# MCG-NJU/MeMOTR

Hardware: AMD Instinct MI355X
Metric: train_frames_per_sec (higher is better)
Workload: dtype f32

## Files before the change

### include/clip_ops_hip.h

```cpp
#ifndef CLIP_OPS_HIP_H
#define CLIP_OPS_HIP_H

#include <stdint.h>

#ifdef __cplusplus
extern "C" {
#endif

#define CLIPOPS_ABI_VERSION 12

int clipops_abi_version(void);
const char *clipops_last_error(void);

int clipops_match_cost_f32(const float *logits, long logit_sl, long logit_sq, const float *boxes, long box_sl,
                           long box_sq, const int64_t *gt_labels, const float *gt_boxes, int n_layers, int Q, int K,
                           int T, float w_class, float w_bbox, float w_giou, float *cost, void *stream);

int clipops_pair_box_loss_fwd_f32(const float *boxes, const int64_t *lay, const int64_t *qidx, long row_mul,
                                  long row_add, const float *tgt_boxes, const int64_t *gidx, const float *weight,
                                  int n, float *l1, float *giou_loss, void *stream);
int clipops_pair_box_loss_bwd_f32(const float *boxes, const int64_t *lay, const int64_t *qidx, long row_mul,
                                  long row_add, const float *tgt_boxes, const int64_t *gidx, const float *weight,
                                  int n, const float *grad_l1, const float *grad_giou, float *grad_boxes,
                                  void *stream);
// ... 55 lines not shown

#define CLIPOPS_ASSIGN_MAX_DIM 2048
int clipops_assign_f32(const float *cost, long stride_problem, long stride_row, long stride_col, int n_problems,
                       int n_rows, int n_cols, int32_t *row_ind, int32_t *col_ind, int32_t *status, void *stream);

int clipops_shift_relu_f32(float *x, const float *shift, const float *res, long planes, int C, long HW, void *stream);
int clipops_shift_relu_bf16(uint16_t *x, const float *shift, const uint16_t *res, long planes, int C, long HW,
                            void *stream);

int clipops_linear_bwd_f32(const float *grad_y, const float *y_relu, const float *x, const float *w, int rows,
                           int in_features, int out_features, float *grad_x, float *grad_w, float *grad_b,
                           void *stream);

int clipops_linear_fwd_f32(const float *x, const float *w, const float *bias, int rows, int in_features,
                           int out_features, int relu, float *y, void *stream);

int clipops_relu_bwd_colsum_partial_f32(const float *g, const float *y, long rows, int cols, int chunk_rows, float *g2,
                                        float *partial, void *stream);

int clipops_result_rows_f32(const float *boxes, const float *scores, const int64_t *ids, const int64_t *labels, int n,
                            int K, int64_t frame, float ori_w, float ori_h, float score_thresh, float area_thresh,
                            float *rows_f, int64_t *rows_i, int32_t *counters, int capacity, void *stream);

#ifdef __cplusplus
}
#endif
#endif
```

### memotr_amd/_clip_lib.py

```python
from __future__ import annotations

import ctypes

from . import _cabi

LIB_PATH = _cabi.lib_path("libclip_ops_hip.so")

ABI_VERSION = 12

c_int, c_long, c_float, c_void_p = ctypes.c_int, ctypes.c_long, ctypes.c_float, ctypes.c_void_p

_PAIR = [c_void_p, c_void_p, c_void_p, c_long, c_long, c_void_p, c_void_p, c_void_p, c_int]
_FOCAL = [c_void_p, c_long, c_long, c_void_p, c_int, c_int, c_int, c_float, c_float]

SYMBOLS = {
    "clipops_abi_version": ([], c_int),
    "clipops_last_error": ([], ctypes.c_char_p),
    "clipops_match_cost_f32": ([c_void_p, c_long, c_long, c_void_p, c_long, c_long, c_void_p, c_void_p] + [c_int] * 4 +
                               [c_float] * 3 + [c_void_p, c_void_p], c_int),
    "clipops_pair_box_loss_fwd_f32": (_PAIR + [c_void_p, c_void_p, c_void_p], c_int),
    "clipops_pair_box_loss_bwd_f32": (_PAIR + [c_void_p, c_void_p, c_void_p, c_void_p], c_int),
    "clipops_pair_iou_f32": ([c_void_p, c_void_p, c_void_p, c_int, c_void_p, c_void_p], c_int),
    "clipops_track_ownership_i64": ([c_void_p, c_int, c_void_p, c_int, c_void_p, c_void_p, c_void_p], c_int),
    "clipops_focal_labels_i64": ([c_void_p, c_void_p, c_void_p, c_int, c_void_p, c_int, c_void_p, c_int, c_void_p, c_int,
# ... 9 lines not shown
                                                                                          c_void_p], c_int),
    "clipops_mha_bwd_f32": ([c_void_p] * 3 + [c_long] * 6 + [c_void_p] * 4 + [c_int] * 3 + [c_float] +
                            [c_void_p, c_long, c_long] * 3 + [c_void_p], c_int),
    "clipops_add_layer_norm_fwd_f32": ([c_void_p] * 4 + [c_long, c_float] + [c_void_p] * 4, c_int),
    "clipops_add_layer_norm_bwd_f32": ([c_void_p] * 4 + [c_long, c_int] + [c_void_p] * 3, c_int),
    "clipops_add_layer_norm_pos_fwd_f32": ([c_void_p] * 5 + [c_long, c_float] + [c_void_p] * 5, c_int),
    "clipops_add_layer_norm_fanin_bwd_f32": ([c_void_p] * 6 + [c_long, c_int] + [c_void_p] * 4, c_int),
    "clipops_sine_embed_fwd_f32": ([c_void_p, c_void_p, c_long, c_int, c_int, c_float, c_void_p, c_void_p], c_int),
    "clipops_sine_embed_bwd_f32": ([c_void_p, c_void_p, c_long, c_int, c_int, c_float, c_void_p, c_void_p, c_void_p],
                                   c_int),
    "clipops_inverse_sigmoid_fwd_f32": ([c_void_p, c_long, c_float, c_void_p, c_void_p], c_int),
    "clipops_inverse_sigmoid_bwd_f32": ([c_void_p, c_void_p, c_long, c_float, c_void_p, c_void_p], c_int),
    "clipops_refine_boxes_fwd_f32": ([c_void_p, c_void_p, c_long, c_float, c_void_p, c_void_p], c_int),
    "clipops_linear_bwd_f32": ([c_void_p] * 4 + [c_int] * 3 + [c_void_p] * 4, c_int),
    "clipops_linear_fwd_f32": ([c_void_p] * 3 + [c_int] * 4 + [c_void_p, c_void_p], c_int),
    "clipops_relu_bwd_colsum_partial_f32": ([c_void_p, c_void_p, c_long, c_int, c_int, c_void_p, c_void_p, c_void_p], c_int),
    "clipops_shift_relu_f32": ([c_void_p, c_void_p, c_void_p, c_long, c_int, c_long, c_void_p], c_int),
    "clipops_shift_relu_bf16": ([c_void_p, c_void_p, c_void_p, c_long, c_int, c_long, c_void_p], c_int),
    "clipops_refine_boxes_bwd_f32": ([c_void_p, c_void_p, c_void_p, c_long, c_float, c_void_p, c_void_p, c_void_p],
                                     c_int),
    "clipops_refine_boxes_split_fwd_f32": ([c_void_p, c_void_p, c_long, c_float, c_void_p, c_void_p, c_void_p], c_int),
    "clipops_result_rows_f32": ([c_void_p] * 4 + [c_int, c_int, ctypes.c_int64] + [c_float] * 4 + [c_void_p] * 3 +
                                [c_int, c_void_p], c_int),
}


lib, check = _cabi.bind("libclip_ops_hip.so", "clipops", SYMBOLS, ABI_VERSION)
```

### memotr_amd/csrc/clip_ops.hip

```cpp
#include <hip/hip_runtime.h>
#include <stdint.h>
#include <stdio.h>

#include <atomic>

#include "../../include/clip_ops_hip.h"
#include "assign_core.h"

namespace {

thread_local char g_err[256] = {0};

int fail(int code, const char *msg) {
    snprintf(g_err, sizeof(g_err), "%s", msg);
    return code;
}

int check_launch(const char *what) {
    const hipError_t e = hipGetLastError();
    if (e != hipSuccess) {
        snprintf(g_err, sizeof(g_err), "%s: %s", what, hipGetErrorString(e));
        return (int)e;
    }
    g_err[0] = 0;
// ... 69 lines not shown
                                                               const int64_t *__restrict__ lay,
                                                               const int64_t *__restrict__ qidx, long row_mul,
                                                               long row_add, const float *__restrict__ tgt,
                                                               const int64_t *__restrict__ gidx,
                                                               const float *__restrict__ weight, int n,
                                                               float *__restrict__ l1, float *__restrict__ gl) {
#pragma clang fp contract(off)
    const int i = blockIdx.x * blockDim.x + threadIdx.x;
    if (i >= n) return;
    const float *pb = boxes + (lay[i] * row_mul + row_add + qidx[i]) * 4;
    const float *tb = tgt + (gidx ? gidx[i] : (long)i) * 4;
    const float p0 = pb[0], p1 = pb[1], p2 = pb[2], p3 = pb[3];
    const float t0 = tb[0], t1 = tb[1], t2 = tb[2], t3 = tb[3];
    float a = ((fabsf(p0 - t0) + fabsf(p1 - t1)) + fabsf(p2 - t2)) + fabsf(p3 - t3);
    float g = 1.f - giou_pair(to_xyxy(p0, p1, p2, p3), to_xyxy(t0, t1, t2, t3));
    if (weight) {
        a *= weight[i];
        g *= weight[i];
    }
    l1[i] = a;
    gl[i] = g;
}

__global__ __launch_bounds__(256) void pair_iou_kernel(const float *__restrict__ boxes, const float *__restrict__ tgt,
                                                      const int64_t *__restrict__ gidx, int n,
                                                      float *__restrict__ iou) {
#pragma clang fp contract(off)
    const int i = blockIdx.x * blockDim.x + threadIdx.x;
    if (i >= n) return;
    const float *pb = boxes + (long)i * 4;
    const float *tb = tgt + (gidx ? gidx[i] : (long)i) * 4;
    const Box a = to_xyxy(pb[0], pb[1], pb[2], pb[3]), b = to_xyxy(tb[0], tb[1], tb[2], tb[3]);
    const float iw = fmaxf(fminf(a.x2, b.x2) - fmaxf(a.x1, b.x1), 0.f);
    const float ih = fmaxf(fminf(a.y2, b.y2) - fmaxf(a.y1, b.y1), 0.f);
    const float inter = iw * ih;
    const float uni = (a.x2 - a.x1) * (a.y2 - a.y1) + (b.x2 - b.x1) * (b.y2 - b.y1) - inter;
    iou[i] = inter / uni;
}

__device__ __forceinline__ float dmax_a(float a, float b) { return a > b ? 1.f : (a == b ? 0.5f : 0.f); }
__device__ __forceinline__ float dmin_a(float a, float b) { return a < b ? 1.f : (a == b ? 0.5f : 0.f); }
__device__ __forceinline__ float sgn(float x) { return x > 0.f ? 1.f : (x < 0.f ? -1.f : 0.f); }

__global__ __launch_bounds__(256) void pair_box_loss_bwd_kernel(const float *__restrict__ boxes,
                                                               const int64_t *__restrict__ lay,
                                                               const int64_t *__restrict__ qidx, long row_mul,
                                                               long row_add, const float *__restrict__ tgt,
                                                               const int64_t *__restrict__ gidx,
                                                               const float *__restrict__ weight, int n,
                                                               const float *__restrict__ g_l1,
                                                               const float *__restrict__ g_gl,
                                                               float *__restrict__ grad_boxes) {
    const int i = blockIdx.x * blockDim.x + threadIdx.x;
    if (i >= n) return;
    const long row = lay[i] * row_mul + row_add + qidx[i];
    const float *pb = boxes + row * 4;
    const float *tb = tgt + (gidx ? gidx[i] : (long)i) * 4;
    const float p0 = pb[0], p1 = pb[1], p2 = pb[2], p3 = pb[3];
    const float t0 = tb[0], t1 = tb[1], t2 = tb[2], t3 = tb[3];
    const float w = weight ? weight[i] : 1.f;
// ... 1091 lines not shown
int clipops_focal_labels_i64(const int64_t *lay, const int64_t *q, const int64_t *g, int n_pairs,
                             const int64_t *gt_labels, int n_gt, const int64_t *matched_idx, int n_tracks,
                             const uint8_t *late, int n_layers, int n_det, int K, int64_t *labels, void *stream) {
    if (n_pairs < 0 || n_gt < 0 || n_tracks < 0 || n_layers < 0 || n_det < 0) return fail(1, "clipops_focal_labels_i64: negative count");
    if ((long)n_layers * (n_det + n_tracks) == 0) { g_err[0] = 0; return 0; }
    if (!labels || !late || (n_pairs > 0 && (!lay || !q || !g || !gt_labels)) || (n_tracks > 0 && !matched_idx) ||
        (n_gt > 0 && !gt_labels))
        return fail(1, "clipops_focal_labels_i64: null pointer");
    hipLaunchKernelGGL(focal_labels_kernel, dim3(1), dim3(256), 0, (hipStream_t)stream, lay, q, g, n_pairs, gt_labels, n_gt,
                       matched_idx, n_tracks, late, n_layers, n_det, K, labels);
    return check_launch("focal_labels_kernel");
}

int clipops_pair_iou_f32(const float *boxes, const float *tgt_boxes, const int64_t *gidx, int n, float *iou,
                         void *stream) {
    if (n < 0) return fail(1, "clipops_pair_iou_f32: negative count");
    if (n == 0) { g_err[0] = 0; return 0; }
    if (!boxes || !tgt_boxes || !iou) return fail(1, "clipops_pair_iou_f32: null pointer");
    hipLaunchKernelGGL(pair_iou_kernel, dim3((n + 255) / 256), dim3(256), 0, (hipStream_t)stream, boxes, tgt_boxes,
                       gidx, n, iou);
    return check_launch("pair_iou_kernel");
}

int clipops_focal_fwd_f32(const float *logits, long sl, long sq, const int64_t *labels, int n_layers, int Nq, int K,
                          float alpha, float gamma, float *loss, void *stream) {
    if (n_layers < 0 || Nq < 0 || K <= 0) return fail(1, "clipops_focal_fwd_f32: bad dimension");
    if (n_layers == 0) { g_err[0] = 0; return 0; }
    if (!loss || (Nq > 0 && (!logits || !labels))) return fail(1, "clipops_focal_fwd_f32: null pointer");
    hipLaunchKernelGGL(focal_fwd_kernel, dim3(n_layers), dim3(256), 0, (hipStream_t)stream, logits, sl, sq, labels, Nq,
                       K, alpha, gamma, loss);
    return check_launch("focal_fwd_kernel");
}

int clipops_focal_bwd_f32(const float *logits, long sl, long sq, const int64_t *labels, int n_layers, int Nq, int K,
                          float alpha, float gamma, const float *grad_loss, float *grad_logits, void *stream) {
    if (n_layers < 0 || Nq < 0 || K <= 0) return fail(1, "clipops_focal_bwd_f32: bad dimension");
    if ((long)n_layers * Nq == 0) { g_err[0] = 0; return 0; }
    if (!logits || !labels || !grad_loss || !grad_logits) return fail(1, "clipops_focal_bwd_f32: null pointer");
    hipLaunchKernelGGL(focal_bwd_kernel, dim3(grid_for((long)n_layers * Nq * K)), dim3(256), 0, (hipStream_t)stream,
                       logits, sl, sq, labels, n_layers, Nq, K, alpha, gamma, grad_loss, grad_logits);
    return check_launch("focal_bwd_kernel");
}

int clipops_sine_embed_fwd_f32(const float *pos, const float *dim_t, long n, int K, int F, float scale, float *out,
                               void *stream) {
    if (n < 0 || K <= 0 || F <= 0) return fail(1, "clipops_sine_embed_fwd_f32: bad dimension");
// ... 303 lines not shown
```

### memotr_amd/engine.py

```python
from __future__ import annotations

import contextlib

from typing import Dict, List, Tuple

import os

import torch
import torch.nn as nn

from .models.utils import get_model
from .structures.track_instances import TrackInstances
from .utils.nested_tensor import tensor_list_to_nested_tensor


def get_param_groups(config: dict, model: nn.Module) -> Tuple[List[Dict], List[str]]:
    def has(name, keys):
        return any(k in name for k in keys)

    backbone, points, updater = ["backbone.backbone"], ["reference_points", "sampling_offsets"], ["query_updater"]
    named = [(n, p) for n, p in model.named_parameters() if p.requires_grad]
    groups = [
        {"params": [p for n, p in named if has(n, backbone)], "lr": config["LR_BACKBONE"]},
        {"params": [p for n, p in named if has(n, points)], "lr": config["LR_POINTS"]},
# ... 151 lines not shown
            if lo + n >= clip_len:
                feats = None
        else:
            batch_frames = frames(lo, lo + n)
            batch_frames.encode_slot = ci
            enc = model(frame=batch_frames, stage="encode")
        if n == 1:
            encoded[lo] = dict(enc, frame_slot=lo, clip_key=clip_key)
            return
        per_frame = {k: (v.split(n_clips, dim=0) if k in ("memory", "valid_ratios", "mask_flatten") else None)
                     for k, v in enc.items()}
        for j in range(n):
            encoded[lo + j] = {k: (per_frame[k][j] if per_frame[k] is not None else v) for k, v in enc.items()}
            encoded[lo + j]["frame_slot"] = lo + j
            encoded[lo + j]["clip_key"] = clip_key

    upd = getattr(core, "query_updater", None)
    hint = (chunks is not None and upd is not None and core.training and getattr(upd, "tp_drop_ratio", 1.0) == 0.0
            and getattr(upd, "fp_insert_ratio", 1.0) == 0.0 and os.environ.get("MEMOTR_KEEP_ROWS", "1") != "0")
    criterion.keep_threshold = upd.update_threshold if hint else None
    if upd is not None:
        upd.__dict__["_keep_rows_ok"] = hint

    def set_up():
        tr = TrackInstances.init_tracks(batch=batch, hidden_dim=core.hidden_dim, num_classes=core.num_classes,
                                        device=device, use_dab=use_dab)
        criterion.init_a_clip(batch=batch, hidden_dim=core.hidden_dim, num_classes=core.num_classes, device=device)
        return tr

    resident = all(v.device.type == torch.device(device).type for v in batch["infos"][0][0].values()
                   if torch.is_tensor(v))
    tracks = None if resident else set_up()
    if chunks is not None:
        encode_chunk(0)
    if tracks is None:
        tracks = set_up()
    owed = None
    for frame_idx in range(clip_len):
        if lazy and frame_idx in starts and frame_idx > 0:
            encode_chunk(starts.index(frame_idx))
        if chunks is None:
            frozen = bool(no_grad_frames) and frame_idx < no_grad_frames
            with (torch.no_grad() if frozen else contextlib.nullcontext()):
                res = model(frame=frames(frame_idx, frame_idx + 1), tracks=tracks)
                previous, new, unmatched = criterion.process_single_frame(model_outputs=res,
                                                                          tracked_instances=tracks,
                                                                          frame_idx=frame_idx)
                if frozen and frame_idx < clip_len - 1:
                    tracks = core.postprocess_single_frame(previous, new, unmatched,
                                                           no_augment=frame_idx < no_grad_frames - 1)
            if frozen:
                continue
        else:
            if frame_idx in on_side:
                torch.cuda.current_stream().wait_stream(side)
                on_side.difference_update(range(frame_idx, clip_len))
            res = model(tracks=tracks, encoded=encoded.pop(frame_idx))
            pending = criterion.begin_frame(model_outputs=res, tracked_instances=tracks, frame_idx=frame_idx)
            if not lazy and frame_idx in starts and starts.index(frame_idx) + 1 < len(chunks):
                encode_chunk(starts.index(frame_idx) + 1)
            if DEFER_LOSSES:
                if owed is not None:
                    criterion.finish_losses(owed)
                previous, new, unmatched = criterion.finish_tracks(pending)
                owed = pending
            else:
                previous, new, unmatched = criterion.finish_frame(pending)
        if frame_idx < clip_len - 1:
            tracks = core.postprocess_single_frame(previous, new, unmatched,
                                                   **({} if chunks is None else {"frame_slot": frame_idx,
                                                                                 "clip_key": clip_key}))
    if owed is not None:
        criterion.finish_losses(owed)
    loss_dict, _ = criterion.get_mean_by_n_gts(with_log=os.environ.get("MEMOTR_LOSS_LOG_SYNC", "0") == "1")
    loss = criterion.get_sum_loss_dict(loss_dict=loss_dict)
    if backward:
        with (torch.autocast(device_type=torch.device(device).type, enabled=False)
              if torch.is_autocast_enabled() else contextlib.nullcontext()):
            (loss / accumulation_steps).backward()
    return loss, loss_dict

# ... 12 lines not shown
```

### memotr_amd/functions/clip_ops.py

```python
from __future__ import annotations

import os

import torch
import torch.nn.functional as F


def fused(*tensors) -> bool:
    return (os.environ.get("MEMOTR_FUSED_CLIP_OPS", "1") != "0"
            and all(t.is_cuda and (t.dtype == torch.float32 or not t.is_floating_point()) for t in tensors))


def config_key() -> tuple:
    return (os.environ.get("MEMOTR_FUSED_CLIP_OPS", "1"), os.environ.get("MEMOTR_COLSUM_TALL", "1"),
            os.environ.get("MEMOTR_ATTN_KERNELS", "1"), os.environ.get("MEMOTR_FUSED_LN", "1"),
            os.environ.get("MEMOTR_FUSED_SHIFT_RELU", "1"), os.environ.get("MEMOTR_FUSED_LINEAR_BWD", "1"),
            os.environ.get("MEMOTR_FUSED_LINEAR_FWD", "1"))


def _lib():
    from .. import _clip_lib
    return _clip_lib


# ... 136 lines not shown
    return out


def assign(cost: torch.Tensor):
    if cost.dim() != 3 or cost.dtype != torch.float32 or not cost.is_cuda:
        raise RuntimeError("assign expects a float32 CUDA tensor of shape (problems, rows, cols)")
    P, R, C = cost.shape
    k = min(R, C)
    row = torch.empty((P, k), dtype=torch.int32, device=cost.device)
    col = torch.empty((P, k), dtype=torch.int32, device=cost.device)
    status = torch.empty((P,), dtype=torch.int32, device=cost.device)
    L = _lib()
    L.check(L.lib.clipops_assign_f32(cost.data_ptr(), cost.stride(0), cost.stride(1), cost.stride(2), P, R, C,
                                     row.data_ptr(), col.data_ptr(), status.data_ptr(), _stream(cost)),
            "clipops_assign_f32")
    return row, col, status


def pair_iou_reference(boxes, tgt_boxes, gidx=None):
    from ..models.criterion import paired_iou
    from ..utils.box_ops import box_cxcywh_to_xyxy
    tb = tgt_boxes if gidx is None else tgt_boxes[gidx]
    return paired_iou(box_cxcywh_to_xyxy(boxes), box_cxcywh_to_xyxy(tb))


class _FocalPerLayer(torch.autograd.Function):
    @staticmethod
    def forward(ctx, logits, labels, alpha, gamma):
        n_layers, Nq, K = logits.shape
        sl, sq = _strides3(logits)
        loss = torch.empty((n_layers,), dtype=torch.float32, device=logits.device)
        L = _lib()
        L.check(L.lib.clipops_focal_fwd_f32(logits.data_ptr(), sl, sq, labels.data_ptr(), n_layers, Nq, K, alpha, gamma,
                                            loss.data_ptr(), _stream(logits)), "clipops_focal_fwd_f32")
        ctx.save_for_backward(logits, labels)
        ctx.alpha, ctx.gamma = alpha, gamma
        return loss

    @staticmethod
    def backward(ctx, g):
        logits, labels = ctx.saved_tensors
        n_layers, Nq, K = logits.shape
        sl, sq = _strides3(logits)
        grad = torch.empty((n_layers, Nq, K), dtype=torch.float32, device=logits.device)
        L = _lib()
        L.check(L.lib.clipops_focal_bwd_f32(logits.data_ptr(), sl, sq, labels.data_ptr(), n_layers, Nq, K, ctx.alpha,
# ... 496 lines not shown
```

### memotr_amd/models/criterion.py

```python
from __future__ import annotations

import os
from typing import Dict, List, Tuple

import numpy as np
import torch
import torch.distributed
import torch.nn.functional as F

from ..functions import clip_ops
from ..structures.track_instances import TrackInstances
from ..utils.box_ops import box_cxcywh_to_xyxy, box_iou_union, generalized_box_iou
from ..utils.utils import distributed_world_size, is_distributed
from .matcher import HungarianMatcher
from .matcher import build as build_matcher
from .utils import logits_to_scores

_LOSS_KEYS = ("box_l1_loss", "box_giou_loss", "label_focal_loss")



def batch_item(x: torch.Tensor, b: int) -> torch.Tensor:
    return x.squeeze(0) if x.shape[0] == 1 else x[b]


def rows_of(x: torch.Tensor, b: int, idx: torch.Tensor) -> torch.Tensor:
    return batch_item(x, b).index_select(0, idx)


def upload(values, dtype, device):
    t = torch.as_tensor(values, dtype=dtype)
    if torch.device(device).type == "cuda":
        return t.pin_memory().to(device, non_blocking=True)
    return t.to(device)


def _fp32_island(fn):
    import functools

    @functools.wraps(fn)
    def wrapped(self, *args, **kwargs):
        if torch.is_autocast_enabled():
            with torch.autocast(device_type="cuda", enabled=False):
                return fn(self, *args, **kwargs)
        return fn(self, *args, **kwargs)
    return wrapped


_MAX_CLIP_FRAMES = 63

# ... 223 lines not shown
            n_fl = state["n_flag_list"][b]
            flags_h.append(host[pos:pos + n_fl].bool().numpy() if n_fl else None)
            pos += n_fl
            free_h = host[pos:pos + n_gt].bool().numpy()
            pos += n_gt
            cost_h = host[pos:pos + n_layers * nd * n_gt].view(n_layers, nd, n_gt).numpy()
            pos += n_layers * nd * n_gt
            free_idx = free_h.nonzero()[0]
            for li in range(n_layers):
                if early[li]:
                    qi, gj = self.matcher.solve(cost_h[li])
                else:
                    qi, tj = self.matcher.solve(cost_h[li][:, free_idx])
                    gj = free_idx[tj]
                rows_layer[b].append(np.full((len(qi),), li, dtype=np.int64))
                rows_q[b].append(qi)
                rows_g[b].append(gj)
                if li == 0:
                    main_q.append((qi, gj))

        new_tracks, unmatched = [], []
        n_det_out = len(model_outputs["det_query_embed"])
        per_clip = []
        for b in range(B):
            tr, gt = tracked_instances[b], gts[b]
            n_tr = len(tr)
            n_main = len(main_q[b][0])
            mq, mg = (np.asarray(x, dtype=np.int64) for x in main_q[b])
            unclaimed = np.ones((n_det_out,), dtype=bool)
            unclaimed[mq] = False
            free_np = np.flatnonzero(unclaimed)
            keep_np = None
            if flags_h[b] is not None:
                fl = flags_h[b]
                sc, idf, gtf = fl[:nd + n_tr], fl[nd + n_tr:nd + 2 * n_tr], fl[nd + 2 * n_tr:]
                keep_np = np.concatenate((np.flatnonzero(sc[nd:nd + n_tr] | idf),
                                          n_tr + np.flatnonzero(sc[mq] | gtf[mg]),
                                          n_tr + n_main + np.flatnonzero(sc[free_np])))
            cat = lambda rows: (np.concatenate([np.asarray(r, dtype=np.int64) for r in rows])
                                if rows else np.zeros((0,), dtype=np.int64))
            lay_np, q_np, g_np = cat(rows_layer[b]), cat(rows_q[b]), cat(rows_g[b])
            n_pairs = len(q_np)
            up = upload(np.concatenate((lay_np, q_np, g_np, free_np) + (() if keep_np is None else (keep_np,))),
                        torch.long, dev)
            lay_i, q_i, g_i = up[:n_pairs], up[n_pairs:2 * n_pairs], up[2 * n_pairs:3 * n_pairs]
            free_q = up[3 * n_pairs:3 * n_pairs + len(free_np)]
# ... 26 lines not shown
            d.query_embed = queries if self.use_dab else torch.cat(
                (model_outputs["det_query_embed"][free_q][:, :self.hidden_dim], queries), dim=-1)
            d.ids = -torch.ones((len(free_q),), dtype=torch.long, device=dev)
            d.matched_idx = -torch.ones((len(free_q),), dtype=torch.long, device=dev)
            d.iou = torch.zeros((len(free_q),), dtype=torch.float, device=dev)
            if keep_rows is not None:
                d._keep_rows = (keep_rows, float(self.keep_threshold))
            unmatched.append(d)

            if not tr.on_device(dev):
                tr = tr.to(dev)
            tracked_instances[b] = tr
            if len(gt) > 0:
                iou_of = clip_ops.pair_iou if clip_ops.fused(logits_all, boxes_all, gt.boxes) else clip_ops.pair_iou_reference
                if n_main > 0:
                    nt.iou = iou_of(nt.boxes, gt.boxes, nt.matched_idx)
                if n_tr > 0:
                    has = tr.matched_idx >= 0
                    tr.iou = torch.where(has, iou_of(tr.boxes, gt.boxes, tr.matched_idx.clamp(min=0)), tr.iou)
            new_tracks.append(nt)
        self.n_gts.append(sum(n_gt_list))
        state["per_clip"] = per_clip
        return tracked_instances, new_tracks, unmatched

    @_fp32_island
    def finish_losses(self, state: dict):
        frame_idx, early, logits_all, boxes_all = state["frame_idx"], state["early"], state["logits_all"], state["boxes_all"]
        nd, dev, n_layers = self.n_det_queries, self.device, len(state["layers"])
        gts = self.gt_trackinstances_list[frame_idx]
        loss_label = torch.zeros((n_layers,), device=dev)
        loss_l1 = torch.zeros((n_layers,), device=dev)
        loss_giou = torch.zeros((n_layers,), device=dev)
        for b, clip in enumerate(state.pop("per_clip")):
            gt, n_tr, matched_idx = gts[b], clip["n_tr"], clip["matched_idx"]
            lay_i, q_i, g_i = clip["idx"]
            n_q = nd + n_tr
            late = self._constant(("late", tuple(early)), [not e for e in early], torch.bool, dev)
            has = matched_idx >= 0 if n_tr > 0 else None
            if (clip_ops.fused(logits_all, boxes_all, gt.boxes) and gt.labels.dtype == torch.int64
                    and os.environ.get("MEMOTR_FUSED_BOOKKEEPING", "1") != "0"):
                labels = clip_ops.focal_labels(lay_i, q_i, g_i, gt.labels, matched_idx, late, nd, n_tr, self.num_classes)
            else:
                labels = clip_ops.focal_labels_reference(lay_i, q_i, g_i, gt.labels, matched_idx, late, nd, n_tr,
                                                         self.num_classes)
            use_kernels = clip_ops.fused(logits_all, boxes_all, gt.boxes)
            if use_kernels:
# ... 129 lines not shown
```

### memotr_amd/models/query_updater.py

```python
from __future__ import annotations

from typing import List, Optional

import torch
import torch.nn as nn

from ..structures.track_instances import TrackInstances
from ..utils.box_ops import box_cxcywh_to_xyxy, box_iou_union
from ..functions.clip_ops import add_layer_norm
from ..modules.attention import memory_attention
from ..utils.utils import inverse_sigmoid
from .ffn import FFN
from .mlp import MLP
from .utils import logits_to_scores, pos_to_pos_embed


PACKED_TRACKS = __import__("os").environ.get("MEMOTR_PACKED_TRACKS", "1") != "0"


class QueryUpdater(nn.Module):
    def __init__(self, hidden_dim: int, ffn_dim: int, tp_drop_ratio: float, fp_insert_ratio: float, dropout: float,
                 use_checkpoint: bool, use_dab: bool, update_threshold: float, long_memory_lambda: float,
                 visualize: bool = False):
        super().__init__()
# ... 109 lines not shown
        f = TrackInstances(frame_height=1.0, frame_width=1.0, hidden_dim=C).to(device=device)
        rn = lambda *s: torch.randn(s, dtype=torch.float, device=device)
        f.query_embed = rn(1, C if self.use_dab else 2 * C)
        f.output_embed = rn(1, C)
        f.ref_pts = rn(1, 4)
        f.ids = torch.as_tensor([-2], dtype=torch.long, device=device)
        f.matched_idx = torch.as_tensor([-2], dtype=torch.long, device=device)
        f.boxes = rn(1, 4)
        f.logits = rn(1, n_logits)
        f.iou = torch.zeros((1,), dtype=torch.float, device=device)
        f.last_output = rn(1, C)
        f.long_memory = rn(1, C)
        return f

    def select_active_tracks(self, previous_tracks, new_tracks, unmatched_dets, no_augment: bool = False):
        cat = TrackInstances.cat_tracked_instances
        if not self.training:
            assert len(previous_tracks) == 1 and len(new_tracks) == 1
            self._seed_memories(new_tracks[0])
            active = cat(previous_tracks[0], new_tracks[0])
            return [active[active.ids >= 0]]
        tracks = []
        for b in range(len(new_tracks)):
            self._seed_memories(new_tracks[b])
            self._seed_memories(unmatched_dets[b])
            if self.tp_drop_ratio == 0.0 and self.fp_insert_ratio == 0.0:
                active = (TrackInstances.cat_packed if PACKED_TRACKS else cat)(previous_tracks[b], new_tracks[b],
                                                                               unmatched_dets[b])
                keep_rows, keep_thr = unmatched_dets[b].__dict__.pop("_keep_rows", None) or (None, None)
                if (keep_rows is not None and self.__dict__.get("_keep_rows_ok", False)
                        and keep_thr == float(self.update_threshold)):
                    active = active[keep_rows]
                else:
                    scores = torch.max(logits_to_scores(active.logits), dim=1).values
                    active = active[(scores > self.update_threshold) | (active.ids >= 0)]
                active.ids = torch.where(active.iou < 0.5, torch.full_like(active.ids, -1), active.ids)
            else:
                active = cat(previous_tracks[b], new_tracks[b])
                active = active[(active.iou > 0.5) & (active.ids >= 0)]
                if self.tp_drop_ratio > 0.0 and not no_augment and len(active) > 0:
                    active = active[torch.rand((len(active),)) > self.tp_drop_ratio]
                if self.fp_insert_ratio > 0.0 and not no_augment:
                    picked = active[torch.bernoulli(torch.ones((len(active),)) * self.fp_insert_ratio).bool()]
                    if len(unmatched_dets[b]) > 0 and len(picked) > 0:
                        if len(picked) >= len(unmatched_dets[b]):
                            fp = unmatched_dets[b]
# ... 19 lines not shown
```

Measured before the change: 41.78.

## Fuse track handover gather into a single HIP kernel with custom backward

Adds a fused handover path in which the criterion builds the next frame's active track set directly. A per-row HIP kernel copies logits, boxes, refs, memories and queries into one packed buffer and computes IoU, ids and matched indices, with a matching backward kernel that scatters gradients. This replaces many small torch gathers, concatenations and the separate select-active-tracks filtering in the query updater, cutting kernel launches and host overhead per frame. It adds a cross-module contract (the _keep_rows handover) that raises an error if the thresholds or augmentation settings differ.

```diff
diff --git a/include/clip_ops_hip.h b/include/clip_ops_hip.h
--- a/include/clip_ops_hip.h
+++ b/include/clip_ops_hip.h
@@ -101,6 +101,38 @@
                             int K, int64_t frame, float ori_w, float ori_h, float score_thresh, float area_thresh,
                             float *rows_f, int64_t *rows_i, int32_t *counters, int capacity, void *stream);
 
+enum {
+    CLIPOPS_HO_LOGITS = 0,
+    CLIPOPS_HO_BOXES,
+    CLIPOPS_HO_OUTPUTS,
+    CLIPOPS_HO_QUERIES,
+    CLIPOPS_HO_LAST_REF,
+    CLIPOPS_HO_INIT_REF,
+    CLIPOPS_HO_DET_EMBED,
+    CLIPOPS_HO_PREV_REF,
+    CLIPOPS_HO_PREV_LONG,
+    CLIPOPS_HO_PREV_LAST,
+    CLIPOPS_HO_PREV_QUERY,
+    CLIPOPS_HO_PREV_IOU,
+    CLIPOPS_HO_N_SOURCES
+};
+typedef struct {
+    const float *ptr[CLIPOPS_HO_N_SOURCES];
+    long row_stride[CLIPOPS_HO_N_SOURCES];
+} clipops_handover_sources;
+typedef struct {
+    float *ptr[CLIPOPS_HO_N_SOURCES];
+} clipops_handover_grads;
+
+int clipops_handover_fwd_f32(const clipops_handover_sources *src, const int64_t *prev_ids, const int64_t *prev_matched,
+                             const float *gt_boxes, const int64_t *gt_ids, const int64_t *table, int n_keep, int n_det,
+                             int n_tracks, int n_gt, int K, int C, int use_dab, float *base, int64_t *ids,
+                             int64_t *matched_idx, void *stream);
+
+int clipops_handover_bwd_f32(const float *grad_base, const int64_t *table, const int64_t *inv_q, const int64_t *inv_prev,
+                             int n_keep, int n_q, int n_det, int n_tracks, int K, int C, int use_dab, int det_cols,
+                             const clipops_handover_grads *grad, void *stream);
+
 #ifdef __cplusplus
 }
 #endif
diff --git a/memotr_amd/_clip_lib.py b/memotr_amd/_clip_lib.py
--- a/memotr_amd/_clip_lib.py
+++ b/memotr_amd/_clip_lib.py
@@ -55,7 +55,20 @@
     "clipops_refine_boxes_split_fwd_f32": ([c_void_p, c_void_p, c_long, c_float, c_void_p, c_void_p, c_void_p], c_int),
     "clipops_result_rows_f32": ([c_void_p] * 4 + [c_int, c_int, ctypes.c_int64] + [c_float] * 4 + [c_void_p] * 3 +
                                 [c_int, c_void_p], c_int),
+    "clipops_handover_fwd_f32": ([c_void_p] * 6 + [c_int] * 7 + [c_void_p] * 4, c_int),
+    "clipops_handover_bwd_f32": ([c_void_p] * 4 + [c_int] * 8 + [c_void_p, c_void_p], c_int),
 }
+
+HANDOVER_SOURCES = ("logits", "boxes", "outputs", "queries", "last_ref", "init_ref", "det_embed", "prev_ref",
+                    "prev_long", "prev_last", "prev_query", "prev_iou")
+
+
+class HandoverSources(ctypes.Structure):
+    _fields_ = [("ptr", c_void_p * len(HANDOVER_SOURCES)), ("row_stride", c_long * len(HANDOVER_SOURCES))]
+
+
+class HandoverGrads(ctypes.Structure):
+    _fields_ = [("ptr", c_void_p * len(HANDOVER_SOURCES))]
 
 
 lib, check = _cabi.bind("libclip_ops_hip.so", "clipops", SYMBOLS, ABI_VERSION)
diff --git a/memotr_amd/csrc/clip_ops.hip b/memotr_amd/csrc/clip_ops.hip
--- a/memotr_amd/csrc/clip_ops.hip
+++ b/memotr_amd/csrc/clip_ops.hip
@@ -115,6 +115,15 @@
     gl[i] = g;
 }
 
+__device__ __forceinline__ float iou_pair(const Box a, const Box b) {
+#pragma clang fp contract(off)
+    const float iw = fmaxf(fminf(a.x2, b.x2) - fmaxf(a.x1, b.x1), 0.f);
+    const float ih = fmaxf(fminf(a.y2, b.y2) - fmaxf(a.y1, b.y1), 0.f);
+    const float inter = iw * ih;
+    const float uni = (a.x2 - a.x1) * (a.y2 - a.y1) + (b.x2 - b.x1) * (b.y2 - b.y1) - inter;
+    return inter / uni;
+}
+
 __global__ __launch_bounds__(256) void pair_iou_kernel(const float *__restrict__ boxes, const float *__restrict__ tgt,
                                                       const int64_t *__restrict__ gidx, int n,
                                                       float *__restrict__ iou) {
@@ -123,12 +132,173 @@
     if (i >= n) return;
     const float *pb = boxes + (long)i * 4;
     const float *tb = tgt + (gidx ? gidx[i] : (long)i) * 4;
-    const Box a = to_xyxy(pb[0], pb[1], pb[2], pb[3]), b = to_xyxy(tb[0], tb[1], tb[2], tb[3]);
-    const float iw = fmaxf(fminf(a.x2, b.x2) - fmaxf(a.x1, b.x1), 0.f);
-    const float ih = fmaxf(fminf(a.y2, b.y2) - fmaxf(a.y1, b.y1), 0.f);
-    const float inter = iw * ih;
-    const float uni = (a.x2 - a.x1) * (a.y2 - a.y1) + (b.x2 - b.x1) * (b.y2 - b.y1) - inter;
-    iou[i] = inter / uni;
+    iou[i] = iou_pair(to_xyxy(pb[0], pb[1], pb[2], pb[3]), to_xyxy(tb[0], tb[1], tb[2], tb[3]));
+}
+
+struct HandoverCols {
+    int K, C, QW, oB, oR, oO, oM, oS, oQ, oI, W;
+};
+
+HandoverCols handover_cols(int K, int C, int use_dab) {
+    HandoverCols c;
+    c.K = K;
+    c.C = C;
+    c.QW = use_dab ? C : 2 * C;
+    c.oB = K;
+    c.oR = K + 4;
+    c.oO = K + 8;
+    c.oM = c.oO + C;
+    c.oS = c.oM + C;
+    c.oQ = c.oS + C;
+    c.oI = c.oQ + c.QW;
+    c.W = c.oI + 1;
+    return c;
+}
+
+__device__ __forceinline__ void row_copy(float *__restrict__ dst, const float *__restrict__ src, int n) {
+    for (int c = threadIdx.x; c < n; c += blockDim.x) dst[c] = src[c];
+}
+__device__ __forceinline__ void row_sum(float *__restrict__ dst, const float *__restrict__ a,
+                                        const float *__restrict__ b, int n) {
+    for (int c = threadIdx.x; c < n; c += blockDim.x) dst[c] = a[c] + b[c];
+}
+__device__ __forceinline__ void row_zero(float *__restrict__ dst, int n) {
+    for (int c = threadIdx.x; c < n; c += blockDim.x) dst[c] = 0.f;
+}
+
+__global__ __launch_bounds__(256) void handover_fwd_kernel(clipops_handover_sources src,
+                                                          const int64_t *__restrict__ prev_ids,
+                                                          const int64_t *__restrict__ prev_matched,
+                                                          const float *__restrict__ gt_boxes,
+                                                          const int64_t *__restrict__ gt_ids,
+                                                          const int64_t *__restrict__ table, int n_det, int n_tracks,
+                                                          int n_gt, int use_dab, HandoverCols cols,
+                                                          float *__restrict__ base, int64_t *__restrict__ ids,
+                                                          int64_t *__restrict__ matched_idx) {
+    const int o = blockIdx.x;
+    const int64_t kind = table[3 * (long)o], s = table[3 * (long)o + 1];
+    int64_t g = table[3 * (long)o + 2];
+    float *row = base + (long)o * cols.W;
+    bool ok;
+    if (kind == 0) {
+        ok = s >= 0 && s < n_tracks;
+        if (ok) {
+            g = prev_matched[s];
+            ok = g >= -1 && g < n_gt;
+        }
+    } else {
+        ok = (kind == 1 || kind == 2) && s >= 0 && s < n_det && (kind == 2 || (g >= 0 && g < n_gt));
+    }
+    if (!ok) {
+        row_zero(row, cols.W);
+        if (threadIdx.x == 0) ids[o] = matched_idx[o] = -1;
+        return;
+    }
+    const long m = kind == 0 ? (long)n_det + s : s;
+#define HO_ROW(i, r) (src.ptr[i] + (r) * src.row_stride[i])
+    const float *box = HO_ROW(CLIPOPS_HO_BOXES, m);
+    row_copy(row, HO_ROW(CLIPOPS_HO_LOGITS, m), cols.K);
+    row_copy(row + cols.oB, box, 4);
+    row_copy(row + cols.oO, HO_ROW(CLIPOPS_HO_OUTPUTS, m), cols.C);
+    if (kind == 0) {
+        row_copy(row + cols.oR, HO_ROW(CLIPOPS_HO_PREV_REF, s), 4);
+        row_copy(row + cols.oM, HO_ROW(CLIPOPS_HO_PREV_LONG, s), cols.C);
+        row_copy(row + cols.oS, HO_ROW(CLIPOPS_HO_PREV_LAST, s), cols.C);
+        row_copy(row + cols.oQ, HO_ROW(CLIPOPS_HO_PREV_QUERY, s), cols.QW);
+    } else {
+        row_copy(row + cols.oR, HO_ROW(kind == 1 ? CLIPOPS_HO_LAST_REF : CLIPOPS_HO_INIT_REF, s), 4);
+        row_copy(row + cols.oM, HO_ROW(CLIPOPS_HO_QUERIES, s), cols.C);
+        row_copy(row + cols.oS, HO_ROW(CLIPOPS_HO_OUTPUTS, s), cols.C);
+        if (use_dab) {
+            row_copy(row + cols.oQ, HO_ROW(CLIPOPS_HO_QUERIES, s), cols.C);
+        } else {
+            row_copy(row + cols.oQ, HO_ROW(CLIPOPS_HO_DET_EMBED, s), cols.C);
+            row_copy(row + cols.oQ + cols.C, HO_ROW(CLIPOPS_HO_QUERIES, s), cols.C);
+        }
+    }
+    if (threadIdx.x == 0) {
+        float iou = 0.f;
+        int64_t id = -1;
+        if (kind == 2) {
+            g = -1;
+        } else {
+            if (g >= 0) {
+                const float *tb = gt_boxes + g * 4;
+                iou = iou_pair(to_xyxy(box[0], box[1], box[2], box[3]), to_xyxy(tb[0], tb[1], tb[2], tb[3]));
+            } else {
+                iou = HO_ROW(CLIPOPS_HO_PREV_IOU, s)[0];
+            }
+            id = kind == 0 ? prev_ids[s] : gt_ids[g];
+        }
+        row[cols.oI] = iou;
+        ids[o] = iou < 0.5f ? (int64_t)-1 : id;
+        matched_idx[o] = g;
+    }
+#undef HO_ROW
+}
+
+__global__ __launch_bounds__(256) void handover_bwd_kernel(const float *__restrict__ grad_base,
+                                                          const int64_t *__restrict__ table,
+                                                          const int64_t *__restrict__ inv_q,
+                                                          const int64_t *__restrict__ inv_prev, int n_keep, int n_q,
+                                                          int n_det, int n_tracks, int use_dab, int det_cols,
+                                                          HandoverCols cols, clipops_handover_grads grad) {
+    const int C = cols.C;
+    if ((int)blockIdx.x < n_q) {
+        const long r = blockIdx.x;
+        int64_t o = inv_q[r], kind = -1;
+        if (o >= 0 && o < n_keep) {
+            kind = table[3 * o];
+            const int64_t s = table[3 * o + 1];
+            const bool back = kind == 0 ? (s >= 0 && s < n_tracks && n_det + s == r)
+                                        : ((kind == 1 || kind == 2) && s == r && r < n_det);
+            if (!back) kind = -1;
+        }
+        const float *gr = kind >= 0 ? grad_base + o * cols.W : nullptr;
+        float *g_out = grad.ptr[CLIPOPS_HO_OUTPUTS], *g_qry = grad.ptr[CLIPOPS_HO_QUERIES];
+        float *g_last = grad.ptr[CLIPOPS_HO_LAST_REF], *g_init = grad.ptr[CLIPOPS_HO_INIT_REF];
+        float *g_det = grad.ptr[CLIPOPS_HO_DET_EMBED];
+        if (g_out) {
+            if (kind == 0) row_copy(g_out + r * C, gr + cols.oO, C);
+            else if (kind > 0) row_sum(g_out + r * C, gr + cols.oO, gr + cols.oS, C);
+            else row_zero(g_out + r * C, C);
+        }
+        if (g_qry) {
+            if (kind > 0) row_sum(g_qry + r * C, gr + cols.oQ + (use_dab ? 0 : C), gr + cols.oM, C);
+            else row_zero(g_qry + r * C, C);
+        }
+        if (g_last) {
+            if (kind == 1) row_copy(g_last + r * 4, gr + cols.oR, 4);
+            else row_zero(g_last + r * 4, 4);
+        }
+        if (g_init) {
+            if (kind == 2) row_copy(g_init + r * 4, gr + cols.oR, 4);
+            else row_zero(g_init + r * 4, 4);
+        }
+        if (g_det && !use_dab && r < n_det) {
+            if (kind > 0) {
+                row_copy(g_det + r * det_cols, gr + cols.oQ, C);
+                row_zero(g_det + r * det_cols + C, det_cols - C);
+            } else {
+                row_zero(g_det + r * det_cols, det_cols);
+            }
+        }
+        return;
+    }
+    const long j = (long)blockIdx.x - n_q;
+    if (j >= n_tracks) return;
+    int64_t o = inv_prev[j];
+    if (!(o >= 0 && o < n_keep && table[3 * o] == 0 && table[3 * o + 1] == j)) o = -1;
+    const float *gr = o >= 0 ? grad_base + o * cols.W : nullptr;
+    float *g_ref = grad.ptr[CLIPOPS_HO_PREV_REF], *g_long = grad.ptr[CLIPOPS_HO_PREV_LONG];
+    float *g_lo = grad.ptr[CLIPOPS_HO_PREV_LAST], *g_qe = grad.ptr[CLIPOPS_HO_PREV_QUERY];
+    if (g_ref) { if (gr) row_copy(g_ref + j * 4, gr + cols.oR, 4); else row_zero(g_ref + j * 4, 4); }
+    if (g_long) { if (gr) row_copy(g_long + j * C, gr + cols.oM, C); else row_zero(g_long + j * C, C); }
+    if (g_lo) { if (gr) row_copy(g_lo + j * C, gr + cols.oS, C); else row_zero(g_lo + j * C, C); }
+    if (g_qe) {
+        if (gr) row_copy(g_qe + j * cols.QW, gr + cols.oQ, cols.QW);
+        else row_zero(g_qe + j * cols.QW, cols.QW);
+    }
 }
 
 __device__ __forceinline__ float dmax_a(float a, float b) { return a > b ? 1.f : (a == b ? 0.5f : 0.f); }
@@ -1266,6 +1436,47 @@
     return check_launch("pair_iou_kernel");
 }
 
+int clipops_handover_fwd_f32(const clipops_handover_sources *src, const int64_t *prev_ids, const int64_t *prev_matched,
+                             const float *gt_boxes, const int64_t *gt_ids, const int64_t *table, int n_keep, int n_det,
+                             int n_tracks, int n_gt, int K, int C, int use_dab, float *base, int64_t *ids,
+                             int64_t *matched_idx, void *stream) {
+    if (n_keep < 0 || n_det < 0 || n_tracks < 0 || n_gt < 0) return fail(1, "clipops_handover_fwd_f32: negative size");
+    if (K < 1 || C < 1) return fail(1, "clipops_handover_fwd_f32: K < 1 or C < 1");
+    if (n_keep == 0) { g_err[0] = 0; return 0; }
+    if (!src || !table || !base || !ids || !matched_idx || (n_gt > 0 && (!gt_boxes || !gt_ids)))
+        return fail(1, "clipops_handover_fwd_f32: null pointer");
+    for (int i = 0; i < CLIPOPS_HO_N_SOURCES; ++i) {
+        const bool prev = i >= CLIPOPS_HO_PREV_REF;
+        const bool needed = prev ? n_tracks > 0 : (i == CLIPOPS_HO_DET_EMBED ? (!use_dab && n_det > 0) : n_det + n_tracks > 0);
+        if (needed && !src->ptr[i]) return fail(1, "clipops_handover_fwd_f32: null source pointer");
+        if (needed && src->row_stride[i] < 0) return fail(1, "clipops_handover_fwd_f32: negative row stride");
+    }
+    if (n_tracks > 0 && (!prev_ids || !prev_matched)) return fail(1, "clipops_handover_fwd_f32: null pointer");
+    hipLaunchKernelGGL(handover_fwd_kernel, dim3(n_keep), dim3(256), 0, (hipStream_t)stream, *src, prev_ids,
+                       prev_matched, gt_boxes, gt_ids, table, n_det, n_tracks, n_gt, use_dab,
+                       handover_cols(K, C, use_dab), base, ids, matched_idx);
+    return check_launch("handover_fwd_kernel");
+}
+
+int clipops_handover_bwd_f32(const float *grad_base, const int64_t *table, const int64_t *inv_q, const int64_t *inv_prev,
+                             int n_keep, int n_q, int n_det, int n_tracks, int K, int C, int use_dab, int det_cols,
+                             const clipops_handover_grads *grad, void *stream) {
+    if (n_keep < 0 || n_q < 0 || n_det < 0 || n_tracks < 0) return fail(1, "clipops_handover_bwd_f32: negative size");
+    if (K < 1 || C < 1) return fail(1, "clipops_handover_bwd_f32: K < 1 or C < 1");
+    if ((long)n_det + n_tracks > n_q) return fail(1, "clipops_handover_bwd_f32: n_q < n_det + n_tracks");
+    if (n_q + n_tracks == 0) { g_err[0] = 0; return 0; }
+    if (!grad || !inv_q || (n_tracks > 0 && !inv_prev) || (n_keep > 0 && (!grad_base || !table)))
+        return fail(1, "clipops_handover_bwd_f32: null pointer");
+    if (grad->ptr[CLIPOPS_HO_LOGITS] || grad->ptr[CLIPOPS_HO_BOXES] || grad->ptr[CLIPOPS_HO_PREV_IOU])
+        return fail(1, "clipops_handover_bwd_f32: logits, boxes and iou take no gradient");
+    if (grad->ptr[CLIPOPS_HO_DET_EMBED] && (use_dab || det_cols < C))
+        return fail(1, "clipops_handover_bwd_f32: det_embed gradient under DAB or narrower than C");
+    hipLaunchKernelGGL(handover_bwd_kernel, dim3(n_q + n_tracks), dim3(256), 0, (hipStream_t)stream, grad_base, table,
+                       inv_q, inv_prev, n_keep, n_q, n_det, n_tracks, use_dab, det_cols, handover_cols(K, C, use_dab),
+                       *grad);
+    return check_launch("handover_bwd_kernel");
+}
+
 int clipops_focal_fwd_f32(const float *logits, long sl, long sq, const int64_t *labels, int n_layers, int Nq, int K,
                           float alpha, float gamma, float *loss, void *stream) {
     if (n_layers < 0 || Nq < 0 || K <= 0) return fail(1, "clipops_focal_fwd_f32: bad dimension");
diff --git a/memotr_amd/engine.py b/memotr_amd/engine.py
--- a/memotr_amd/engine.py
+++ b/memotr_amd/engine.py
@@ -197,6 +197,8 @@
     if upd is not None:
         upd.__dict__["_keep_rows_ok"] = hint
 
+    handover = (hint and torch.device(device).type == "cuda" and os.environ.get("MEMOTR_FUSED_HANDOVER", "1") != "0")
+
     def set_up():
         tr = TrackInstances.init_tracks(batch=batch, hidden_dim=core.hidden_dim, num_classes=core.num_classes,
                                         device=device, use_dab=use_dab)
@@ -232,6 +234,7 @@
                 on_side.difference_update(range(frame_idx, clip_len))
             res = model(tracks=tracks, encoded=encoded.pop(frame_idx))
             pending = criterion.begin_frame(model_outputs=res, tracked_instances=tracks, frame_idx=frame_idx)
+            pending["handover"], pending["gather"] = handover, frame_idx < clip_len - 1
             if not lazy and frame_idx in starts and starts.index(frame_idx) + 1 < len(chunks):
                 encode_chunk(starts.index(frame_idx) + 1)
             if DEFER_LOSSES:
diff --git a/memotr_amd/functions/clip_ops.py b/memotr_amd/functions/clip_ops.py
--- a/memotr_amd/functions/clip_ops.py
+++ b/memotr_amd/functions/clip_ops.py
@@ -1,5 +1,6 @@
 from __future__ import annotations
 
+import ctypes
 import os
 
 import torch
@@ -182,6 +183,159 @@
     from ..utils.box_ops import box_cxcywh_to_xyxy
     tb = tgt_boxes if gidx is None else tgt_boxes[gidx]
     return paired_iou(box_cxcywh_to_xyxy(boxes), box_cxcywh_to_xyxy(tb))
+
+
+HANDOVER_CARRIED, HANDOVER_NEW, HANDOVER_UNCLAIMED = 0, 1, 2
+HANDOVER_DIFF = ("outputs", "queries", "last_ref", "init_ref", "det_embed", "prev_ref", "prev_long", "prev_last",
+                 "prev_query")
+
+
+def handover_tables(n_det: int, n_q: int, n_tracks: int, new_q, new_g, free_q, keep):
+    import numpy as np
+    n_new, n_free = len(new_q), len(free_q)
+    kind = np.concatenate((np.full((n_tracks,), HANDOVER_CARRIED, dtype=np.int64),
+                           np.full((n_new,), HANDOVER_NEW, dtype=np.int64),
+                           np.full((n_free,), HANDOVER_UNCLAIMED, dtype=np.int64)))
+    src = np.concatenate((np.arange(n_tracks, dtype=np.int64), np.asarray(new_q, dtype=np.int64),
+                          np.asarray(free_q, dtype=np.int64)))
+    gt = np.concatenate((np.full((n_tracks,), -1, dtype=np.int64), np.asarray(new_g, dtype=np.int64),
+                         np.full((n_free,), -1, dtype=np.int64)))
+    keep = np.asarray(keep, dtype=np.int64)
+    table = np.stack((kind[keep], src[keep], gt[keep]), axis=1)
+    rows = np.arange(len(keep), dtype=np.int64)
+    carried = table[:, 0] == HANDOVER_CARRIED
+    inv_q = np.full((n_q,), -1, dtype=np.int64)
+    inv_q[np.where(carried, n_det + table[:, 1], table[:, 1])] = rows
+    inv_prev = np.full((n_tracks,), -1, dtype=np.int64)
+    inv_prev[table[carried, 1]] = rows[carried]
+    return np.concatenate((table.reshape(-1), inv_q, inv_prev))
+
+
+def _handover_views(tables, n_keep, n_q, n_tracks):
+    table = tables[:3 * n_keep]
+    inv_q = tables[3 * n_keep:3 * n_keep + n_q]
+    inv_prev = tables[3 * n_keep + n_q:3 * n_keep + n_q + n_tracks]
+    return table, inv_q, inv_prev
+
+
+def _rows_dense(t):
+    return t if t.dim() == 2 and (t.shape[1] == 1 or t.stride(1) == 1) and t.stride(0) >= 0 else t.contiguous()
+
+
+class _Handover(torch.autograd.Function):
+    @staticmethod
+    def forward(ctx, outputs, queries, last_ref, init_ref, det_embed, prev_ref, prev_long, prev_last, prev_query,
+                logits, boxes, prev_iou, prev_ids, prev_matched, gt_boxes, gt_ids, tables, n_keep, n_det):
+        L = _lib()
+        use_dab = det_embed is None
+        n_q, C, K = outputs.shape[0], outputs.shape[1], logits.shape[1]
+        n_tracks, n_gt = prev_ref.shape[0], gt_boxes.shape[0]
+        QW = C if use_dab else 2 * C
+        named = dict(logits=logits, boxes=boxes, outputs=outputs, queries=queries, last_ref=last_ref, init_ref=init_ref,
+                     det_embed=det_embed, prev_ref=prev_ref, prev_long=prev_long, prev_last=prev_last,
+                     prev_query=prev_query, prev_iou=prev_iou.reshape(-1, 1))
+        widths = dict(logits=K, boxes=4, outputs=C, queries=C, last_ref=4, init_ref=4, det_embed=C, prev_ref=4,
+                      prev_long=C, prev_last=C, prev_query=QW, prev_iou=1)
+        src, keep = L.HandoverSources(), []
+        for i, name in enumerate(L.HANDOVER_SOURCES):
+            t = named[name]
+            if t is None or t.shape[0] == 0:
+                continue
+            lead = n_tracks if name.startswith("prev_") else (n_det if name == "det_embed" else n_det + n_tracks)
+            if t.dtype != torch.float32 or t.dim() != 2 or t.shape[0] < lead or (
+                    t.shape[1] != widths[name] and not (name == "det_embed" and t.shape[1] >= C)):
+                raise RuntimeError(f"handover: source {name} has shape {tuple(t.shape)} ({t.dtype})")
+            t = _rows_dense(t.detach())
+            keep.append(t)
+            src.ptr[i], src.row_stride[i] = t.data_ptr(), t.stride(0)
+        if n_q != queries.shape[0] or n_q != last_ref.shape[0] or n_q != init_ref.shape[0]:
+            raise RuntimeError("handover: the model-output sources differ in their row counts")
+        if tables.dtype != torch.int64 or tables.numel() != 3 * n_keep + n_q + n_tracks:
+            raise RuntimeError("handover: the table does not have 3 * n_keep + n_q + n_tracks int64 entries")
+        tables = tables.contiguous()
+        prev_ids, prev_matched, gt_boxes, gt_ids = (t.contiguous() for t in (prev_ids, prev_matched, gt_boxes, gt_ids))
+        if n_tracks and (prev_ids.shape[0] != n_tracks or prev_matched.shape[0] != n_tracks):
+            raise RuntimeError("handover: ids / matched_idx of the previous set do not have one entry per track")
+        dev = outputs.device
+        base = torch.empty((n_keep, K + 8 + 3 * C + QW + 1), dtype=torch.float32, device=dev)
+        ints = torch.empty((2, n_keep), dtype=torch.int64, device=dev)
+        L.check(L.lib.clipops_handover_fwd_f32(
+            ctypes.byref(src), prev_ids.data_ptr() if n_tracks else None, prev_matched.data_ptr() if n_tracks else None,
+            gt_boxes.data_ptr(), gt_ids.data_ptr(), tables.data_ptr(), n_keep, n_det, n_tracks, n_gt, K, C,
+            int(use_dab), base.data_ptr(), ints[0].data_ptr(), ints[1].data_ptr(), _stream(outputs)),
+            "clipops_handover_fwd_f32")
+        ctx.save_for_backward(tables)
+        ctx.dims = (n_keep, n_q, n_det, n_tracks, K, C, use_dab, 0 if det_embed is None else det_embed.shape[1], QW)
+        ctx.mark_non_differentiable(ints)
+        return base, ints
+
+    @staticmethod
+    def backward(ctx, g_base, _g_ints):
+        L = _lib()
+        (tables,) = ctx.saved_tensors
+        n_keep, n_q, n_det, n_tracks, K, C, use_dab, det_cols, QW = ctx.dims
+        table, inv_q, inv_prev = _handover_views(tables, n_keep, n_q, n_tracks)
+        g_base = g_base.contiguous()
+        shapes = dict(outputs=(n_q, C), queries=(n_q, C), last_ref=(n_q, 4), init_ref=(n_q, 4),
+                      det_embed=(n_det, det_cols), prev_ref=(n_tracks, 4), prev_long=(n_tracks, C),
+                      prev_last=(n_tracks, C), prev_query=(n_tracks, QW))
+        wanted = [name for i, name in enumerate(HANDOVER_DIFF) if ctx.needs_input_grad[i]]
+        flat = torch.empty((sum(shapes[n][0] * shapes[n][1] for n in wanted),), dtype=torch.float32, device=g_base.device)
+        grads, out, pos = L.HandoverGrads(), {}, 0
+        for name in wanted:
+            r, c = shapes[name]
+            out[name] = flat[pos:pos + r * c].view(r, c)
+            pos += r * c
+            if r * c:
+                grads.ptr[L.HANDOVER_SOURCES.index(name)] = out[name].data_ptr()
+        if flat.numel():
+            L.check(L.lib.clipops_handover_bwd_f32(
+                g_base.data_ptr(), table.data_ptr(), inv_q.data_ptr(), inv_prev.data_ptr() if n_tracks else None,
+                n_keep, n_q, n_det, n_tracks, K, C, int(use_dab), det_cols, ctypes.byref(grads), _stream(g_base)),
+                "clipops_handover_bwd_f32")
+        return tuple(out.get(name) for name in HANDOVER_DIFF) + (None,) * 10
+
+
+def handover(outputs, queries, last_ref, init_ref, det_embed, prev_ref, prev_long, prev_last, prev_query, logits, boxes,
+             prev_iou, prev_ids, prev_matched, gt_boxes, gt_ids, tables, n_keep: int, n_det: int):
+    base, ints = _Handover.apply(outputs, queries, last_ref, init_ref, det_embed, prev_ref, prev_long, prev_last,
+                                 prev_query, logits, boxes, prev_iou, prev_ids, prev_matched, gt_boxes, gt_ids, tables,
+                                 n_keep, n_det)
+    return base, ints[0], ints[1]
+
+
+def handover_reference(outputs, queries, last_ref, init_ref, det_embed, prev_ref, prev_long, prev_last, prev_query,
+                       logits, boxes, prev_iou, prev_ids, prev_matched, gt_boxes, gt_ids, tables, n_keep: int,
+                       n_det: int):
+    n_q, C = outputs.shape
+    n_tracks = prev_ref.shape[0]
+    table, _, _ = _handover_views(tables, n_keep, n_q, n_tracks)
+    kind, s, g = table.view(n_keep, 3).unbind(1)
+    carried, new = (kind == HANDOVER_CARRIED), (kind == HANDOVER_NEW)
+    m = torch.where(carried, n_det + s, s)
+    q = torch.where(carried, torch.zeros_like(s), s)
+
+    def prev(t):
+        width = 1 if t.dim() == 1 else t.shape[1]
+        if n_tracks == 0:
+            return t.new_zeros((n_keep, width))
+        return t.reshape(n_tracks, width)[torch.where(carried, s, torch.zeros_like(s))]
+
+    col = carried[:, None]
+    det_q = queries[q] if det_embed is None else torch.cat((det_embed[q][:, :C], queries[q]), dim=-1)
+    box = boxes[m]
+    ref = torch.where(col, prev(prev_ref), torch.where(new[:, None], last_ref[q], init_ref[q]))
+    g_own = torch.where(carried, prev(prev_matched).reshape(-1), g)
+    iou_gt = pair_iou_reference(box.detach(), gt_boxes, g_own.clamp(min=0))
+    iou = torch.where(carried, torch.where(g_own >= 0, iou_gt, prev(prev_iou).reshape(-1)),
+                      torch.where(new, iou_gt, torch.zeros_like(iou_gt)))
+    ids = torch.where(carried, prev(prev_ids).reshape(-1), torch.where(new, gt_ids[g.clamp(min=0)], torch.full_like(g, -1)))
+    base = torch.cat((logits[m].detach(), box.detach(), ref, outputs[m], torch.where(col, prev(prev_long), queries[q]),
+                      torch.where(col, prev(prev_last), outputs[q]), torch.where(col, prev(prev_query), det_q),
+                      iou[:, None]), dim=1)
+    ids = torch.where(iou < 0.5, torch.full_like(ids, -1), ids)
+    matched = torch.where(carried, g_own, torch.where(new, g, torch.full_like(g, -1)))
+    return base, ids, matched
 
 
 class _FocalPerLayer(torch.autograd.Function):
diff --git a/memotr_amd/models/criterion.py b/memotr_amd/models/criterion.py
--- a/memotr_amd/models/criterion.py
+++ b/memotr_amd/models/criterion.py
@@ -9,7 +9,7 @@
 import torch.nn.functional as F
 
 from ..functions import clip_ops
-from ..structures.track_instances import TrackInstances
+from ..structures.track_instances import TrackInstances, _empty
 from ..utils.box_ops import box_cxcywh_to_xyxy, box_iou_union, generalized_box_iou
 from ..utils.utils import distributed_world_size, is_distributed
 from .matcher import HungarianMatcher
@@ -26,6 +26,10 @@
 
 def rows_of(x: torch.Tensor, b: int, idx: torch.Tensor) -> torch.Tensor:
     return batch_item(x, b).index_select(0, idx)
+
+
+def _no_columns(n: int, device) -> torch.Tensor:
+    return _empty((n, 0), device=device)
 
 
 def upload(values, dtype, device):
@@ -295,6 +299,11 @@
         new_tracks, unmatched = [], []
         n_det_out = len(model_outputs["det_query_embed"])
         per_clip = []
+        if state.get("handover", False):
+            counted = self._handover(state, main_q, flags_h, (rows_layer, rows_q, rows_g), state.get("gather", True))
+            if counted is not None:
+                self.n_gts.append(sum(n_gt_list))
+                return (tracked_instances,) + counted
         for b in range(B):
             tr, gt = tracked_instances[b], gts[b]
             n_tr = len(tr)
@@ -367,6 +376,73 @@
         self.n_gts.append(sum(n_gt_list))
         state["per_clip"] = per_clip
         return tracked_instances, new_tracks, unmatched
+
+    def _handover(self, state: dict, main_q, flags_h, rows, gather: bool):
+        model_outputs, tracked, gts = state["model_outputs"], state["tracked_instances"], \
+            self.gt_trackinstances_list[state["frame_idx"]]
+        nd, dev = self.n_det_queries, self.device
+        if os.environ.get("MEMOTR_FUSED_HANDOVER", "1") == "0" or not self.aux_loss:
+            return None
+        n_det_out = len(model_outputs["det_query_embed"])
+        outputs_all = model_outputs["outputs"]
+        plans = []
+        for b, (tr, gt) in enumerate(zip(tracked, gts)):
+            n_tr = len(tr)
+            fl = flags_h[b]
+            mq, mg = (np.asarray(x, dtype=np.int64) for x in main_q[b])
+            if fl is None or len(gt) == 0 or n_det_out != nd:
+                return None
+            unclaimed = np.ones((nd,), dtype=bool)
+            unclaimed[mq] = False
+            free_np = np.flatnonzero(unclaimed)
+            sc, idf, gtf = fl[:nd + n_tr], fl[nd + n_tr:nd + 2 * n_tr], fl[nd + 2 * n_tr:]
+            keep_np = np.concatenate((np.flatnonzero(sc[nd:nd + n_tr] | idf), n_tr + np.flatnonzero(sc[mq] | gtf[mg]),
+                                      n_tr + len(mq) + np.flatnonzero(sc[free_np])))
+            tensors = (batch_item(outputs_all, b), batch_item(model_outputs["pred_bboxes"], b), gt.boxes)
+            if (len(keep_np) == 0 or tr.ids.dtype != torch.int64 or gt.ids.dtype != torch.int64
+                    or any(t.dtype != torch.float32 for t in tensors)
+                    or (outputs_all.is_cuda and not clip_ops.fused(*tensors))):
+                return None
+            plans.append((n_tr, mq, mg, free_np, keep_np))
+        gather_fn = clip_ops.handover if outputs_all.is_cuda else clip_ops.handover_reference
+        C = outputs_all.shape[-1]
+        K = model_outputs["pred_logits"].shape[-1]
+        widths = [K, 4, 4, C, C, C, C if self.use_dab else 2 * C, 1]
+        new_tracks, unmatched, per_clip = [], [], []
+
+        def counted(n, tr):
+            t = TrackInstances(frame_height=tr.frame_height, frame_width=tr.frame_width, device=dev)
+            t.ref_pts = t.query_embed = _no_columns(n, dev)
+            return t
+
+        for b, (n_tr, mq, mg, free_np, keep_np) in enumerate(plans):
+            tr, gt = tracked[b], gts[b]
+            lay_np, q_np, g_np = (np.concatenate([np.asarray(r, dtype=np.int64) for r in rr[b]]) for rr in rows)
+            n_pairs = len(q_np)
+            outputs = batch_item(outputs_all, b)
+            parts = (lay_np, q_np, g_np)
+            if gather:
+                parts += (clip_ops.handover_tables(nd, outputs.shape[0], n_tr, mq, mg, free_np, keep_np),)
+            up = upload(np.concatenate(parts), torch.long, dev)
+            per_clip.append({"idx": (up[:n_pairs], up[n_pairs:2 * n_pairs], up[2 * n_pairs:3 * n_pairs]), "n_tr": n_tr,
+                             "matched_idx": tr.matched_idx if n_tr > 0 else None})
+            new_tracks.append(counted(len(mq), tr))
+            unmatched.append(counted(len(free_np), tr))
+            if not gather:
+                continue
+            base, ids, matched = gather_fn(
+                outputs, batch_item(model_outputs["aux_outputs"][-1]["queries"], b),
+                batch_item(model_outputs["last_ref_pts"], b), batch_item(model_outputs["init_ref_pts"], b),
+                None if self.use_dab else model_outputs["det_query_embed"],
+                tr.ref_pts, tr.long_memory, tr.last_output, tr.query_embed,
+                batch_item(model_outputs["pred_logits"], b), batch_item(model_outputs["pred_bboxes"], b),
+                tr.iou, tr.ids, tr.matched_idx, gt.boxes, gt.ids, up[3 * n_pairs:], len(keep_np), nd)
+            act = TrackInstances(frame_height=tr.frame_height, frame_width=tr.frame_width, device=dev)
+            act._set_packed(base, TrackInstances.PACKED_FLOAT, widths)
+            act.ids, act.matched_idx = ids, matched
+            unmatched[-1]._keep_rows = (act, float(self.keep_threshold))
+        state["per_clip"] = per_clip
+        return new_tracks, unmatched
 
     @_fp32_island
     def finish_losses(self, state: dict):
diff --git a/memotr_amd/models/query_updater.py b/memotr_amd/models/query_updater.py
--- a/memotr_amd/models/query_updater.py
+++ b/memotr_amd/models/query_updater.py
@@ -155,6 +155,15 @@
             return [active[active.ids >= 0]]
         tracks = []
         for b in range(len(new_tracks)):
+            handed = unmatched_dets[b].__dict__.get("_keep_rows", None)
+            if handed is not None and isinstance(handed[0], TrackInstances):
+                del unmatched_dets[b].__dict__["_keep_rows"]
+                if not (self.tp_drop_ratio == 0.0 and self.fp_insert_ratio == 0.0
+                        and self.__dict__.get("_keep_rows_ok", False) and handed[1] == float(self.update_threshold)):
+                    raise RuntimeError("the criterion handed over an active track set gathered for another "
+                                       "selection rule (threshold or augmentation changed within a clip)")
+                tracks.append(handed[0])
+                continue
             self._seed_memories(new_tracks[b])
             self._seed_memories(unmatched_dets[b])
             if self.tp_drop_ratio == 0.0 and self.fp_insert_ratio == 0.0:
```

Result: faster. 42.35, median of 6 (+1.4%).
